# shenwei356/unikmer

Measured on AMD Instinct MI355X. Metric: k-mers/sec for union+inter of 1e9-k-mer k=31 sets, higher is better.
Workload: dtype u64

## Files before the change

unikmer_amd/csrc/ukm_ctx.hip:

```cpp
#include <stdarg.h>
#include <stdlib.h>

#include <algorithm>

#include "ukm_internal.h"

static thread_local char g_err[512] = "";

void ukm_set_error(const char *fmt, ...) {
    va_list ap;
    va_start(ap, fmt);
    vsnprintf(g_err, sizeof(g_err), fmt, ap);
    va_end(ap);
}

extern "C" const char *ukm_last_error(void) { return g_err; }
extern "C" int ukm_version(void) { return 1000 * 0 + 1; }

extern "C" int ukm_device_count(int *n) {
    if (!n) UKM_FAIL(UKM_ERR_INVALID, "ukm_device_count: n is NULL");
    int c = 0;
    hipError_t e = hipGetDeviceCount(&c);
    if (e != hipSuccess) {
        (void)hipGetLastError();
        c = 0;
    }
    *n = c;
    return UKM_OK;
}

extern char **environ;

static const char *const UKM_OPTION_KEYS[] = {
    "punion", "punion_tax", "punion_ranked", "place", "srmerge", "kway", "no_kway", "no_fold", "no_pfold", "pfold_tax", "common_probe",
    "sort_local", "sort_counting", "sort_fan", "win_strip", "nthash_strip", "force_ticket", "setop_src", "setop_defer", "punion_clade", "srmerge_clade",
    "punion_k0", "punion_claim", "punion_debug", "kway_k", "kway_r", "kway_top2", "kway_debug", "srmerge_fill", "srmerge_spr", "srmerge_buckets",
    "srmerge_debug", "fold_debug", "sort_debug", "strip_l", "win_strip_l", "setop_fused_part", "setop_fix",
};

static std::string knob_name(const char *key) {
    std::string n = "UKM_";
    for (const char *p = key; *p; p++) n.push_back((char)toupper((unsigned char)*p));
    return n;
}

const char *ukm_env(const ukm_ctx *c, const char *name) {
    if (c) {
        auto o = c->opts.find(name);
        if (o != c->opts.end()) return o->second.c_str();
        if (!c->env_live) {
            auto k = c->knobs.find(name);
            return k == c->knobs.end() ? nullptr : k->second.c_str();
        }
    }
    return getenv(name);
}

extern "C" int ukm_ctx_set_option(ukm_ctx *c, const char *key, long long value) {
    if (!c || !key) UKM_FAIL(UKM_ERR_INVALID, "ukm_ctx_set_option: NULL argument");
    for (const char *k : UKM_OPTION_KEYS)
        if (strcmp(k, key) == 0) {
            c->opts[knob_name(key)] = std::to_string(value);
            if (strcmp(key, "force_ticket") == 0) c->setop_force_ticket = c->ticket_latched || value != 0;
            return UKM_OK;
        }
    UKM_FAIL(UKM_ERR_INVALID, "ukm_ctx_set_option: unknown option '%s'", key);
}

extern "C" int ukm_ctx_unset_option(ukm_ctx *c, const char *key) {
    if (!c || !key) UKM_FAIL(UKM_ERR_INVALID, "ukm_ctx_unset_option: NULL argument");
    c->opts.erase(knob_name(key));
    if (strcmp(key, "force_ticket") == 0) c->setop_force_ticket = c->ticket_latched || ukm_env_is(c, "UKM_FORCE_TICKET", '1');
    return UKM_OK;
}

extern "C" int ukm_ctx_get_option(ukm_ctx *c, const char *key, long long *value, int *is_set) {
    if (!c || !key || !value || !is_set) UKM_FAIL(UKM_ERR_INVALID, "ukm_ctx_get_option: NULL argument");
    const std::string n = knob_name(key);
    const char *e = ukm_env(c, n.c_str());
    *is_set = (e && *e) ? 1 : 0;
    *value = *is_set ? atoll(e) : 0;
    return UKM_OK;
}

extern "C" int ukm_ctx_get_stat(ukm_ctx *c, const char *key, unsigned long long *value) {
    if (!c || !key || !value) UKM_FAIL(UKM_ERR_INVALID, "ukm_ctx_get_stat: NULL argument");
    if (strcmp(key, "punion_attempts") == 0) *value = c->stat_punion_attempts;
    else if (strcmp(key, "sort_fused_hist") == 0) *value = c->stat_sort_fused_hist;
// ... 37 lines not shown
        if (strncmp(*e, "UKM_", 4) != 0) continue;
        const char *eq = strchr(*e, '=');
        if (eq) c->knobs[std::string(*e, (size_t)(eq - *e))] = std::string(eq + 1);
    }
    c->env_live = ukm_env_is(c, "UKM_ENV_LIVE", '1');
    c->setop_force_ticket = ukm_env_is(c, "UKM_FORCE_TICKET", '1');
    *out = c;
    return UKM_OK;
}

static void ws_free_all(ukm_ctx *c) {
    for (auto &b : c->blocks) (void)hipFree(b.base);
    c->blocks.clear();
}

extern "C" int ukm_ctx_destroy(ukm_ctx *c) {
    if (!c) return UKM_OK;
    (void)hipSetDevice(c->device);
    (void)hipStreamSynchronize(c->stream);
    if (c->comm) (void)ukm_comm_destroy(c);
    ws_free_all(c);
    if (c->tax_parent) (void)hipFree(c->tax_parent);
    if (c->tax_depth) (void)hipFree(c->tax_depth);
    if (c->tax_merged) (void)hipFree(c->tax_merged);
    if (c->tax_anc) (void)hipFree(c->tax_anc);
    if (c->tax_euler) (void)hipFree(c->tax_euler);
    if (c->tax_node_at) (void)hipFree(c->tax_node_at);
    if (c->tax_clade) (void)hipFree(c->tax_clade);
    if (c->tax_clade8) (void)hipFree(c->tax_clade8);
    if (c->tax_pair) (void)hipFree(c->tax_pair);
    if (c->tax_top) (void)hipFree(c->tax_top);
    if (c->h_scratch) (void)hipHostFree(c->h_scratch);
    if (c->sort_stat_dev) (void)hipFree(c->sort_stat_dev);
    if (c->ev_start) (void)hipEventDestroy(c->ev_start);
    if (c->ev_stop) (void)hipEventDestroy(c->ev_stop);
    if (c->ev_k0) (void)hipEventDestroy(c->ev_k0);
    if (c->ev_k1) (void)hipEventDestroy(c->ev_k1);
    if (c->xfer) {
        (void)hipStreamSynchronize(c->xfer);
        (void)hipStreamDestroy(c->xfer);
    }
    if (c->ev_xfer) (void)hipEventDestroy(c->ev_xfer);
    for (int i = 0; i < 2; i++) {
        if (c->side[i]) { (void)hipStreamSynchronize(c->side[i]); (void)hipStreamDestroy(c->side[i]); }
        if (c->ev_side[i]) (void)hipEventDestroy(c->ev_side[i]);
    }
    if (c->ev_fork) (void)hipEventDestroy(c->ev_fork);
    if (c->ev_comp) (void)hipEventDestroy(c->ev_comp);
    if (c->own_stream && c->stream) (void)hipStreamDestroy(c->stream);
    delete c;
    return UKM_OK;
}

extern "C" int ukm_ctx_set_stream(ukm_ctx *c, void *hip_stream) {
    if (!c) UKM_FAIL(UKM_ERR_INVALID, "ukm_ctx_set_stream: ctx is NULL");
    UKM_HIP(hipSetDevice(c->device));
    UKM_HIP(hipStreamSynchronize(c->stream));
    if (c->own_stream && c->stream) (void)hipStreamDestroy(c->stream);
    c->stream = (hipStream_t)hip_stream;
    c->own_stream = false;
    return UKM_OK;
}

extern "C" int ukm_ctx_sync(ukm_ctx *c) {
    if (!c) UKM_FAIL(UKM_ERR_INVALID, "ukm_ctx_sync: ctx is NULL");
    UKM_HIP(hipSetDevice(c->device));
    UKM_HIP(hipStreamSynchronize(c->stream));
    return UKM_OK;
}

static const size_t WS_ALIGN = 256;
static const size_t WS_MIN_BLOCK = (size_t)64 << 20;

static int ws_new_block(ukm_ctx *c, size_t need) {
    size_t total = 0;
    for (auto &b : c->blocks) total += b.cap;
    size_t cap = std::max(need, std::max(WS_MIN_BLOCK, total));
    void *p = nullptr;
    hipError_t e = hipMalloc(&p, cap);
    if (e != hipSuccess && cap > need) {
        (void)hipGetLastError();
        cap = need;
        e = hipMalloc(&p, cap);
    }
    if (e != hipSuccess) {
        (void)hipGetLastError();
        UKM_FAIL(UKM_ERR_NOMEM, "device workspace allocation of %zu bytes failed: %s", cap,
                 hipGetErrorString(e));
    }
    c->blocks.push_back(WsBlock{(char *)p, cap, 0});
    return UKM_OK;
}

int ws_alloc(ukm_ctx *c, size_t bytes, void **out) {
    bytes = (bytes + WS_ALIGN - 1) / WS_ALIGN * WS_ALIGN;
    if (bytes == 0) bytes = WS_ALIGN;
    if (c->blocks.empty() || c->blocks.back().cap - c->blocks.back().used < bytes)
        UKM_TRY(ws_new_block(c, bytes));
    WsBlock &b = c->blocks.back();
    *out = b.base + b.used;
    b.used += bytes;
    size_t used = 0;
    for (auto &x : c->blocks) used += x.used;
    c->ws_high = std::max(c->ws_high, used);
    return UKM_OK;
}
// ... 88 lines not shown
    }
    void *d = nullptr;
    UKM_TRY(ws_alloc(c, bytes, &d));
    c->copybacks.push_back(ukm_ctx::CopyBack{p, d, bytes});
    *dev = d;
    return UKM_OK;
}

void ukm_out_resize(ukm_ctx *c, void *host, size_t bytes) {
    for (auto &cb : c->copybacks)
        if (cb.host == host) cb.bytes = std::min(cb.bytes, bytes);
}

int ukm_inout(ukm_ctx *c, void *p, size_t bytes, void **dev) {
    if (ukm_is_device_ptr(p)) {
        *dev = p;
        return UKM_OK;
    }
    void *d = nullptr;
    UKM_TRY(ws_alloc(c, bytes, &d));
    if (bytes) UKM_HIP(hipMemcpyAsync(d, p, bytes, hipMemcpyHostToDevice, c->stream));
    c->copybacks.push_back(ukm_ctx::CopyBack{p, d, bytes});
    *dev = d;
    return UKM_OK;
}

int ukm_begin(ukm_ctx *c, CallScope *s) {
    if (!c) UKM_FAIL(UKM_ERR_INVALID, "ctx is NULL");
    s->c = c;
    s->top = (c->depth == 0);
    c->depth++;
    if (s->top) {
        hipError_t e = hipSetDevice(c->device);
        if (e != hipSuccess) {
            c->depth--;
            UKM_FAIL(UKM_ERR_HIP, "hipSetDevice(%d): %s", c->device, hipGetErrorString(e));
        }
        c->copybacks.clear();
        (void)hipEventRecord(c->ev_start, c->stream);
        c->ev_valid = false;
        c->evk_valid = false;
    }
    s->mark = ws_mark(c);
    return UKM_OK;
}

int ukm_finish(CallScope *s, int rc) {
    ukm_ctx *c = s->c;
    c->depth--;
    if (!s->top) {
        ws_release(c, s->mark);
        return rc;
    }
    (void)hipEventRecord(c->ev_stop, c->stream);
    c->ev_valid = true;
    if (rc == UKM_OK) {
        for (auto &cb : c->copybacks) {
            if (cb.bytes == 0) continue;
            hipError_t e = hipMemcpyAsync(cb.host, cb.dev, cb.bytes, hipMemcpyDeviceToHost, c->stream);
            if (e != hipSuccess) {
                ukm_set_error("copy-back failed: %s", hipGetErrorString(e));
                rc = UKM_ERR_HIP;
                break;
            }
        }
    }
    hipError_t e = hipStreamSynchronize(c->stream);
    if (e != hipSuccess && rc == UKM_OK) {
        ukm_set_error("stream synchronize failed: %s", hipGetErrorString(e));
        rc = UKM_ERR_HIP;
    }
    c->copybacks.clear();
    ws_reset_top(c);
    return rc;
}

void ukm_switch_to_tickets(ukm_ctx *c, const char *where) {
    if (!c->setop_force_ticket)
        fprintf(stderr, "[unikmer_hip] look-back watchdog fired in %s: workgroups were not dispatched in order on device %d; "
                        "switching this context to ticketed tile ids\n", where, c->device);
    c->ticket_latched = true;
    c->setop_force_ticket = true;
}

int ukm_read_u64(ukm_ctx *c, const u64 *dev, u64 *host, int n) {
    if (n > 64) UKM_FAIL(UKM_ERR_INVALID, "ukm_read_u64: n too large");
    UKM_HIP(hipMemcpyAsync(c->h_scratch, dev, n * sizeof(u64), hipMemcpyDeviceToHost, c->stream));
    UKM_HIP(hipStreamSynchronize(c->stream));
    for (int i = 0; i < n; i++) host[i] = c->h_scratch[i];
    return UKM_OK;
}

int ukm_lb_ctl_alloc(ukm_ctx *c, u64 ntiles, size_t tail, LbCtl *b, u64 *head) {
    const size_t nstat = lb_status_words(ntiles);
    u64 *ctl = head;
    if (head) {
        UKM_TRY(ws_alloc_t(c, nstat + tail, &b->status));
        b->zero_from = b->status;
        b->zero_words = nstat;
    } else {
        UKM_TRY(ws_alloc_t(c, LbCtl::HEAD + nstat + tail, &ctl));
        b->status = ctl + 8;
        b->zero_from = ctl;
        b->zero_words = LbCtl::HEAD + nstat;
    }
    b->result = ctl;
    b->ticket = (u32 *)(ctl + 2);
    b->tail = b->status + nstat;
// ... 137 lines not shown
```

unikmer_amd/csrc/ukm_internal.h:

```cpp
#pragma once

#include <hip/hip_runtime.h>
#include <stdint.h>
#include <stdio.h>
#include <stdlib.h>
#include <string.h>

#include <functional>
#include <map>
#include <string>
#include <vector>

#include "../../include/unikmer_hip.h"

typedef uint64_t u64;
typedef uint32_t u32;
typedef uint8_t u8;

void ukm_set_error(const char *fmt, ...);

#define UKM_FAIL(code, ...)        \
    do {                           \
        ukm_set_error(__VA_ARGS__); \
        return (code);             \
// ... 113 lines not shown
}

int ws_alloc(ukm_ctx *c, size_t bytes, void **out);
template <typename T>
static inline int ws_alloc_t(ukm_ctx *c, size_t n, T **out) {
    void *p = nullptr;
    int rc = ws_alloc(c, n * sizeof(T), &p);
    *out = (T *)p;
    return rc;
}
struct WsMark {
    size_t nblocks;
    size_t used_last;
};
WsMark ws_mark(ukm_ctx *c);
void ws_release(ukm_ctx *c, WsMark m);

bool ukm_is_device_ptr(const void *p);

int ukm_in(ukm_ctx *c, const void *p, size_t bytes, const void **dev);
template <typename T>
static inline int ukm_in_t(ukm_ctx *c, const T *p, size_t n, const T **dev) {
    const void *d = nullptr;
    if (p == nullptr || n == 0) {
        *dev = p;
        if (p == nullptr) return UKM_OK;
    }
    int rc = ukm_in(c, p, n * sizeof(T), &d);
    *dev = (const T *)d;
    return rc;
}
int ukm_out(ukm_ctx *c, void *p, size_t bytes, void **dev);
template <typename T>
static inline int ukm_out_t(ukm_ctx *c, T *p, size_t n, T **dev) {
    void *d = nullptr;
    if (p == nullptr) {
        *dev = nullptr;
        return UKM_OK;
    }
    int rc = ukm_out(c, p, n * sizeof(T), &d);
    *dev = (T *)d;
    return rc;
}
void ukm_out_resize(ukm_ctx *c, void *host, size_t bytes);
int ukm_inout(ukm_ctx *c, void *p, size_t bytes, void **dev);

struct CallScope {
    ukm_ctx *c;
    bool top;
    WsMark mark;
};
int ukm_begin(ukm_ctx *c, CallScope *s);
int ukm_finish(CallScope *s, int rc);

int ukm_read_u64(ukm_ctx *c, const u64 *dev, u64 *host, int n = 1);

static inline TaxDev ukm_taxdev(const ukm_ctx *c) {
    TaxDev t;
    t.parent = c->tax_parent;
    t.depth = c->tax_depth;
    t.merged = c->tax_merged;
    t.anc = c->tax_anc;
    t.euler = c->tax_euler;
    t.node_at = c->tax_node_at;
    t.clade = c->tax_clade;
    t.clade8 = c->tax_clade8;
    t.pair = c->tax_pair;
    t.kp = c->tax_kp;
    {
        const size_t off = (((size_t)c->tax_kp * c->tax_kp) + 3) & ~(size_t)3;
        t.cpath = c->tax_pair ? reinterpret_cast<const uint4 *>(c->tax_pair + off) : nullptr;
        t.cnode = c->tax_pair ? c->tax_pair + off + 4 * TAX_CPATH_ROWS : nullptr;
    }
    t.top = c->tax_top;
    t.nchunks = c->tax_nchunks;
    t.size = c->tax_size;
    return t;
}

#ifndef LB_STRIDE
#define LB_STRIDE 8
#endif
static inline size_t lb_status_words(u64 ntiles) { return (size_t)ntiles * LB_STRIDE; }

struct LbCtl {
    static constexpr size_t HEAD = 8;
    u64 *result = nullptr;
    u32 *ticket = nullptr;
    u64 *status = nullptr;
    u64 *tail = nullptr;
    u64 *zero_from = nullptr;
    size_t zero_words = 0;
};
int ukm_lb_ctl_alloc(ukm_ctx *c, u64 ntiles, size_t tail, LbCtl *b, u64 *head = nullptr);
int ukm_lb_ctl_zero(ukm_ctx *c, const LbCtl &b);

void ukm_switch_to_tickets(ukm_ctx *c, const char *where);

struct LbLaunch {
    const char *err_name;
    const char *warn_name;
    u64 watchdog;
    bool bracket;
    bool ticket_first;
    bool first_zeroed;
};
// ... 26 lines not shown
```

unikmer_amd/csrc/ukm_setops.hip:

```cpp
#include <algorithm>

#include "ukm_device.h"

namespace {

enum { FLAG_DUP = 1, FLAG_UNSORTED = 2, FLAG_TIMEOUT = 4 };

#ifndef SETOP_NT
#define SETOP_NT 512
#endif
#ifndef SETOP_VT
#define SETOP_VT 19
#endif


struct SetopArgs {
    const u64 *a, *b;
    const u32 *ta, *tb;
    const u32 *ra, *rb;
    u64 na, nb;
    u64 *mp;
    u64 *status;
    u32 *ticket;
    u64 *result;
    u64 *out;
    u32 *tout;
    u64 out_cap;
    u64 ntiles;
    TaxDev tax;
    u32 flags;
    u64 *dbg;
    const u64 *na_dev;
    u32 zero_status;
    u32 cta, ctb;
    uint4 *fix;
    u32 *fix_cnt;
};
constexpr u32 FIX_SLOTS = 16;

__device__ __forceinline__ void setop_resolve_sizes(SetopArgs &p, u64 tile_items) {
    if (p.na_dev) {
        p.na = *p.na_dev;
        p.ntiles = (p.na + p.nb + tile_items - 1) / tile_items;
    }
}

#ifdef UKM_PROFILE_PHASES
#define PH(i) do { if (tid == 0) { u64 _t = clock64(); ph[i] += _t - tlast; tlast = _t; } } while (0)
#else
#define PH(i) do {} while (0)
#endif

template <bool RANK>
__device__ __forceinline__ bool key_le(u64 ka, u32 ra, u64 kb, u32 rb) {
    if (RANK) return ka < kb || (ka == kb && ra <= rb);
    return ka <= kb;
}
template <bool RANK>
__device__ __forceinline__ bool key_eq(u64 ka, u32 ra, u64 kb, u32 rb) {
    if (RANK) return ka == kb && ra == rb;
    return ka == kb;
}

#ifndef SETOP_PART_COARSE
#define SETOP_PART_COARSE 64
#endif
#ifndef SETOP_PART_INTERP1
#define SETOP_PART_INTERP1 (1 << 17)
#endif
#ifndef SETOP_PART_INTERP
#define SETOP_PART_INTERP 512
#endif
constexpr int PART_COARSE = SETOP_PART_COARSE;
template <bool RANK, int LEVEL>
__global__ void setop_partition_kernel(SetopArgs p, int tile_items) {
    setop_resolve_sizes(p, (u64)tile_items);
    u64 t = (u64)blockIdx.x * blockDim.x + threadIdx.x;
    if (LEVEL == 1) {
        t *= PART_COARSE;
        if (t > p.ntiles + PART_COARSE - 1) return;
        if (t > p.ntiles) t = p.ntiles;
    } else {
        if (LEVEL == 0 && t < p.zero_status) p.status[t * LB_STRIDE] = 0;
        if (t > p.ntiles) return;
        if (LEVEL == 2 && (t % PART_COARSE == 0 || t == p.ntiles)) return;
    }
    const u64 N = p.na + p.nb;
    u64 diag = t * (u64)tile_items;
    if (diag > N) diag = N;
// ... 41 lines not shown
    u64 t = gid >> 6;
    const int lane = (int)(threadIdx.x & 63);
    if (LEVEL == 1) {
        t *= PART_COARSE;
        if (t > p.ntiles + PART_COARSE - 1) return;
        if (t > p.ntiles) t = p.ntiles;
    } else if (t > p.ntiles) {
        return;
    }
    const u64 N = p.na + p.nb;
    u64 diag = t * (u64)tile_items;
    if (diag > N) diag = N;
    u64 lo = diag > p.nb ? diag - p.nb : 0;
    u64 hi = diag < p.na ? diag : p.na;
#if SETOP_PART_INTERP1
    if (lo < hi) {
        const u64 W = SETOP_PART_INTERP1;
        u64 est = (u64)((double)diag * ((double)p.na / (double)N));
        est = est < lo ? lo : (est > hi ? hi : est);
        const u64 L = est > lo + W ? est - W : lo;
        const u64 R = est + W < hi ? est + W : hi;
        bool pl = true, pr = false;
        if (L > lo) { const u64 j = diag - L; pl = key_le<RANK>(p.a[L - 1], RANK ? p.ra[L - 1] : 0, p.b[j], RANK ? p.rb[j] : 0); }
        if (R < hi) { const u64 j = diag - 1 - R; pr = key_le<RANK>(p.a[R], RANK ? p.ra[R] : 0, p.b[j], RANK ? p.rb[j] : 0); }
        if (L > lo) { if (pl) lo = L; else hi = L - 1; }
        if (R < hi) { if (!pr) hi = R; else lo = R + 1; }
    }
#endif
    while (lo < hi) {
        const u64 span = hi - lo;
        const u64 step_n = span <= 64 ? 1 : 0;
        const u64 cand = step_n ? lo + (u64)lane
                                : lo + (span / 65) * (u64)(lane + 1) + ((span % 65) * (u64)(lane + 1)) / 65;
        const bool active = cand < hi;
        bool le = false;
        if (active) {
            const u64 j = diag - 1 - cand;
            le = key_le<RANK>(p.a[cand], RANK ? p.ra[cand] : 0, p.b[j], RANK ? p.rb[j] : 0);
        }
        const u64 m_le = __ballot(le), m_act = __ballot(active);
        const int n_true = __popcll(m_le);
        const int n_act = __popcll(m_act);
        const u64 c_last_true = __shfl(cand, n_true > 0 ? n_true - 1 : 0, 64);
        const u64 c_first_false = __shfl(cand, n_true < 64 ? n_true : 63, 64);
        const u64 nlo = n_true > 0 ? c_last_true + 1 : lo;
        const u64 nhi = n_true < n_act ? c_first_false : hi;
        lo = nlo;
        hi = nhi;
    }
    if (lane == 0) p.mp[t] = lo;
}

template <bool RANK>
__global__ __launch_bounds__(256) void setop_partition_fused_kernel(SetopArgs p, int tile_items, u32 nclear) {
    __shared__ u64 s_end[2];
    const int tid = (int)threadIdx.x, lane = tid & 63, wave = tid >> 6;
    const u64 c0 = (u64)blockIdx.x * PART_COARSE;
    const u64 c1 = (c0 + PART_COARSE < p.ntiles) ? c0 + PART_COARSE : p.ntiles;
    const u64 N = p.na + p.nb;
    if (tid < PART_COARSE && c0 + (u64)tid < p.ntiles) p.status[(c0 + (u64)tid) * LB_STRIDE] = 0;
    if (blockIdx.x == 0 && tid < (int)nclear) p.result[tid] = 0;
    if (wave < 2) {
        const u64 t = wave == 0 ? c0 : c1;
        u64 diag = t * (u64)tile_items;
        if (diag > N) diag = N;
        u64 lo = diag > p.nb ? diag - p.nb : 0;
        u64 hi = diag < p.na ? diag : p.na;
#if SETOP_PART_INTERP1
        if (lo < hi) {
            const u64 W = SETOP_PART_INTERP1;
            u64 est = (u64)((double)diag * ((double)p.na / (double)N));
            est = est < lo ? lo : (est > hi ? hi : est);
            const u64 L = est > lo + W ? est - W : lo;
            const u64 R = est + W < hi ? est + W : hi;
            bool pl = true, pr = false;
            if (L > lo) { const u64 j = diag - L; pl = key_le<RANK>(p.a[L - 1], RANK ? p.ra[L - 1] : 0, p.b[j], RANK ? p.rb[j] : 0); }
            if (R < hi) { const u64 j = diag - 1 - R; pr = key_le<RANK>(p.a[R], RANK ? p.ra[R] : 0, p.b[j], RANK ? p.rb[j] : 0); }
            if (L > lo) { if (pl) lo = L; else hi = L - 1; }
            if (R < hi) { if (!pr) hi = R; else lo = R + 1; }
        }
#endif
        while (lo < hi) {
            const u64 span = hi - lo;
            const u64 cand = span <= 64 ? lo + (u64)lane
                                        : lo + (span / 65) * (u64)(lane + 1) + ((span % 65) * (u64)(lane + 1)) / 65;
            const bool active = cand < hi;
            bool le = false;
            if (active) {
                const u64 j = diag - 1 - cand;
                le = key_le<RANK>(p.a[cand], RANK ? p.ra[cand] : 0, p.b[j], RANK ? p.rb[j] : 0);
            }
            const u64 m_le = __ballot(le), m_act = __ballot(active);
            const int n_true = __popcll(m_le), n_act = __popcll(m_act);
            const u64 c_last_true = __shfl(cand, n_true > 0 ? n_true - 1 : 0, 64);
            const u64 c_first_false = __shfl(cand, n_true < 64 ? n_true : 63, 64);
            const u64 nlo = n_true > 0 ? c_last_true + 1 : lo;
            const u64 nhi = n_true < n_act ? c_first_false : hi;
            lo = nlo;
            hi = nhi;
        }
        if (lane == 0) {
            s_end[wave] = lo;
            if (wave == 0) p.mp[c0] = lo;
            else if (c1 == p.ntiles) p.mp[c1] = lo;
        }
    }
    __syncthreads();
    const u64 t = c0 + (u64)tid;
    if (tid == 0 || tid >= PART_COARSE || t >= c1) return;
    const u64 l0 = s_end[0], h0 = s_end[1];
    u64 diag = t * (u64)tile_items;
    if (diag > N) diag = N;
    u64 lo = diag > p.nb ? diag - p.nb : 0;
    u64 hi = diag < p.na ? diag : p.na;
// ... 636 lines not shown
    }
}

__global__ __launch_bounds__(256) void setop_taxid_fix_kernel(SetopArgs p) {
    const u64 g = (u64)blockIdx.x * 256 + threadIdx.x;
    const u64 tile = g / FIX_SLOTS;
    if (tile >= p.ntiles) return;
    if (sload_u64(&p.result[1]) & FLAG_TIMEOUT) return;
    if ((u32)(g % FIX_SLOTS) >= p.fix_cnt[tile]) return;
    const uint4 e = p.fix[g];
    const u64 pos = ((u64)e.y << 32) | e.x;
    const uint4 zero4 = make_uint4(0, 0, 0, 0);
    const TaxDev &T = p.tax;
    if (pos < p.out_cap) p.tout[pos] = lca_from_rows(T, e.z, e.w, e.z < T.size ? T.anc[e.z] : zero4, e.w < T.size ? T.anc[e.w] : zero4);
}

__global__ void setop_ct_kernel(SetopArgs p, int op) {
    const u32 a = p.cta, b = p.ctb;
    u32 l;
    if (op == UKM_OP_INTER && (p.flags & UKM_F_MIX_TAXID)) l = a == 0 ? b : (b == 0 ? a : lca_dev(p.tax, a, b));
    else l = lca_dev(p.tax, a, b);
    const bool keep = op == UKM_OP_DIFF && (p.flags & UKM_F_CMP_TAXID) && (a == b || lca_dev(p.tax, b, a) == a);
    p.result[4] = (u64)l | ((u64)(keep ? 1u : 0u) << 32);
}

#ifndef SETOP_WAVES
#define SETOP_WAVES 4
#endif
#ifndef SETOP_WAVES_TAX
#define SETOP_WAVES_TAX 6
#endif
template <int OP, bool TAX, bool RANK, bool TICKET, int NTH, int VT, bool CT = false, bool DEFER = false>
__global__ __launch_bounds__(NTH) __attribute__((amdgpu_waves_per_eu((TAX && RANK) ? 2 : ((TAX && VT <= 8) ? SETOP_WAVES_TAX : SETOP_WAVES), (TAX && RANK) ? 8 : ((TAX && VT <= 8) ? SETOP_WAVES_TAX : SETOP_WAVES))))
void setop_tile_kernel(SetopArgs p) {
    static_assert(!(CT && TAX), "CT: no per-record taxids");
    constexpr int TILE = NTH * VT;
    constexpr int SLOTS = TILE + 8;
    constexpr int NP = TilePairs<NTH, VT>::NP;
    __shared__ __attribute__((aligned(16))) u64 s_keys[SLOTS];
    __shared__ __attribute__((aligned(16))) u32 s_tax[TAX ? SLOTS : 2];
    __shared__ __attribute__((aligned(16))) u32 s_rank[RANK ? SLOTS : 2];
    __shared__ u32 s_scan[NTH / 64 + 1];
    __shared__ u64 s_misc[2];
    __shared__ CladeLdsOpt<TAX> s_clade_tab;
    __shared__ FixLdsOpt<DEFER> s_fix;
    const int tid = (int)threadIdx.x;
    if constexpr (DEFER) {
        if (tid == 0) s_fix.t.n = 0;
    }
#ifdef UKM_PROFILE_PHASES
    u64 ph[8] = {0, 0, 0, 0, 0, 0, 0, 0};
    u64 tlast = clock64();
#endif
    const u64 tile = lb_tile_id<TICKET>(p.ticket, &s_misc[0]);
    PH(0);
    setop_resolve_sizes(p, (u64)TILE);
    if (tile >= p.ntiles) return;
    const TileGeom g = tile_geom<NTH, VT>(p, tile);
    u32 bad = 0;
    bool fast = false;
#ifndef SETOP_NO_FAST
    if (!TAX && !RANK) fast = tile_is_fast<NTH, VT>(p, g);
#endif
    if (fast) {
        tile_dma_fast<NTH, VT>(p, g, tid, s_keys);
        __syncthreads();
        PH(1);
    } else {
        u64 rk[2 * NP];
        u32 rt[2 * NP], rr[2 * NP];
        tile_load<TAX, RANK, NTH, VT>(p, g, tid, rk, rt, rr);
        if constexpr (TAX) clade_lds_load(p.tax, s_clade_tab.t, tid, NTH);
        tile_to_lds<TAX, RANK, NTH, VT>(tid, rk, rt, rr, s_keys, s_tax, s_rank);
        __syncthreads();
        PH(1);
        bad = tile_check_order<RANK, NTH, VT>(g, tid, rk, rr, s_keys, s_rank);
    }
    u64 ok[VT];
    u32 ot[VT];
    u32 tbm[VT];
    u32 need = 0, nneed = 0, qpos = 0;
    u32 mask, amask = 0, mmask = 0;
    int ia0 = 0, ib0 = 0;
    u32 ct_lca = 0;
    bool ct_keep = false;
    if (CT) {
        const u64 w = sload_u64(&p.result[4]);
        ct_lca = (u32)w;
        ct_keep = ((w >> 32) & 1ull) != 0;
    }
#ifdef SETOP_ABL_NOMERGE
    mask = 0xAAAAu | (u32)(tid & 1);
#pragma unroll
    for (int s = 0; s < VT; s++) { ok[s] = s_keys[tid * VT + s]; ot[s] = 0; }
#else
    tile_merge<OP, TAX, RANK, CT, NTH, VT, DEFER>(p, g, tid, s_keys, s_tax, s_rank, ok, ot, mask, amask, mmask, ct_keep, ia0, ib0,
                                           TAX ? reinterpret_cast<const CladeLds *>(&s_clade_tab.t) : nullptr, tbm, need);
#endif
    PH(2);
    u32 tile_total;
    u32 excl;
    {
        constexpr int NW = NTH / 64;
        const u32 v = (u32)__popc(mask) | (DEFER ? (u32)__popc(need) << 16 : 0u);
        const int lane = lane_id(), wave = tid >> 6;
        const u32 incl = wave_incl_scan_u32(v);
        if (lane == 63) s_scan[wave] = incl;
// ... 26 lines not shown
        __syncthreads();
        tile_lca_dense<NTH>(p.tax, s_clade_tab.t, tid, nneed, s_keys + tile_total, s_tax, p.fix ? &s_fix.t : nullptr);
    }
    PH(3);
    if (OP == UKM_OP_MERGE_INTERNAL) {
        if (tid == 0) s_misc[1] = tile * (u64)TILE;
    } else if (tid < 64) {
        bool timed_out = false;
#ifdef LB_PRE_SLEEP
        __builtin_amdgcn_s_sleep(LB_PRE_SLEEP);
#endif
#ifdef SETOP_ABL_NOLB
        const u64 base = tile * (u64)TILE;
#else
        const u64 base = lb_resolve(p.status, tile, (u64)tile_total, lane_id(), TICKET ? nullptr : &timed_out);
#endif
        if (tid == 0) s_misc[1] = base;
        if (timed_out) bad |= FLAG_TIMEOUT;
    }
    PH(4);
    if (OP == UKM_OP_MERGE_INTERNAL) bad &= ~FLAG_DUP;
    {
        u32 wbad = 0;
#pragma unroll
        for (u32 f = 1; f <= FLAG_TIMEOUT; f <<= 1)
            if (__ballot((bad & f) != 0)) wbad |= f;
        if (wbad && lane_id() == 0) atomicOr((unsigned long long *)&p.result[1], (unsigned long long)wbad);
    }
    __syncthreads();
    const u64 base = s_misc[1];
    if constexpr (DEFER) {
        if (p.fix) {
            const u32 nf = s_fix.t.n < FIX_SLOTS ? s_fix.t.n : FIX_SLOTS;
            if ((u32)tid < nf) {
                const u64 pos = base + s_fix.t.w[tid];
                p.fix[tile * FIX_SLOTS + (u32)tid] = make_uint4((u32)pos, (u32)(pos >> 32), s_fix.t.a[tid], s_fix.t.b[tid]);
            }
            if (tid == 0) p.fix_cnt[tile] = nf;
        }
    }
#ifndef SETOP_ABL_NOFLUSH
    tile_flush<TAX, NTH>(p, tid, base, tile_total, s_keys, s_tax);
    if (CT) {
        if (p.ta != nullptr || p.tb != nullptr)
            tile_flush_src<OP, NTH, VT>(p, tid, base, tile_total, excl, mask, amask, mmask, ia0, ib0, reinterpret_cast<u32 *>(s_keys));
        else
            tile_flush_ct<OP, NTH, VT>(p, tid, base, tile_total, excl, mask, amask, mmask, ct_lca, reinterpret_cast<u32 *>(s_keys));
    }
#endif
    if (tid == 0 && tile == p.ntiles - 1) p.result[0] = base + tile_total;
    PH(5);
#ifdef UKM_PROFILE_PHASES
    if (tid == 0 && p.dbg) {
        for (int i = 0; i < 7; i++) p.dbg[blockIdx.x * 8 + i] = ph[i];
        p.dbg[blockIdx.x * 8 + 7] = 1;
    }
#endif
}

__global__ void rank_in_run_kernel(const u64 *k, u64 n, u32 *rank) {
    u64 i = (u64)blockIdx.x * blockDim.x + threadIdx.x;
    if (i >= n) return;
    const u64 key = k[i];
    u32 r = 0;
    while (r < 32 && i > r && k[i - r - 1] == key) r++;
    if (r == 32 && i > r && k[i - r - 1] == key) {
        u64 lo = 0, hi = i - 32;
        while (lo < hi) {
            u64 mid = (lo + hi) >> 1;
            if (k[mid] < key) lo = mid + 1; else hi = mid;
        }
        r = (u32)(i - lo);
    }
    rank[i] = r;
}

__global__ void lower_bound_kernel(const u64 *k, u64 n, const u64 *q, int nq, u64 *out) {
    int i = blockIdx.x * blockDim.x + threadIdx.x;
    if (i >= nq) return;
    u64 key = q[i], lo = 0, hi = n;
    while (lo < hi) {
        u64 mid = (lo + hi) >> 1;
        if (k[mid] < key) lo = mid + 1; else hi = mid;
    }
    out[i] = lo;
}

template <int OP, bool TAX, bool RANK, int NTH, int VT, bool CT = false, bool DEFER = false>
void launch_tile(const SetopArgs &p, hipStream_t st, bool ticket) {
    if (CT) hipLaunchKernelGGL(setop_ct_kernel, dim3(1), dim3(1), 0, st, p, OP);
    if (ticket)
        hipLaunchKernelGGL((setop_tile_kernel<OP, TAX, RANK, true, NTH, VT, CT, DEFER>), dim3((unsigned)p.ntiles), dim3(NTH), 0, st, p);
    else
        hipLaunchKernelGGL((setop_tile_kernel<OP, TAX, RANK, false, NTH, VT, CT, DEFER>), dim3((unsigned)p.ntiles), dim3(NTH), 0, st, p);
    if constexpr (DEFER) {
        if (p.fix) hipLaunchKernelGGL(setop_taxid_fix_kernel, dim3((unsigned)((p.ntiles * FIX_SLOTS + 255) / 256)), dim3(256), 0, st, p);
    }
    if constexpr (CT && !RANK) {
        if (p.ta != nullptr || p.tb != nullptr)
            hipLaunchKernelGGL((setop_taxid_gather_kernel<OP, NTH * VT>), dim3((unsigned)p.ntiles), dim3(GATHER_NT), 0, st, p);
    }
}

template <bool TAX, bool RANK, int NTH, int VT, bool CT = false, bool DEFER = false>
void launch_op(int op, const SetopArgs &p, hipStream_t st, bool ticket) {
    if (op == UKM_OP_UNION) launch_tile<UKM_OP_UNION, TAX, RANK, NTH, VT, CT, DEFER>(p, st, ticket);
    else if (op == UKM_OP_INTER) launch_tile<UKM_OP_INTER, TAX, RANK, NTH, VT, CT, DEFER>(p, st, ticket);
    else if (op == UKM_OP_MERGE_INTERNAL) {
        if constexpr (!RANK) launch_tile<UKM_OP_MERGE_INTERNAL, TAX, false, NTH, VT, CT>(p, st, ticket);
    } else launch_tile<UKM_OP_DIFF, TAX, RANK, NTH, VT, CT>(p, st, ticket);
}

constexpr int NTS = SETOP_NT;
constexpr int VT_PLAIN = SETOP_VT;
#ifndef SETOP_VT_TAX
#define SETOP_VT_TAX 7
#endif
constexpr int VT_TAX = SETOP_VT_TAX;
constexpr int VT_RANK = 12;

int run_setop_pass(ukm_ctx *c, int op, const u64 *a, const u32 *ta, const u32 *ra, u64 na,
                   const u64 *b, const u32 *tb, const u32 *rb, u64 nb, bool tax, u32 flags,
                   u64 *out, u32 *tout, u64 out_cap, u64 result_host[2], u32 cta = 0, u32 ctb = 0) {
    const bool rank = ra != nullptr;
    bool ct = tax && !ta && !tb;
    const bool defer_form = SETOP_TAX_DEFER != 0 && c->tax_pair != nullptr && !ukm_env_is(c, "UKM_SETOP_DEFER", '0');
    const int src_mode = ukm_env_int(c, "UKM_SETOP_SRC", defer_form ? 0 : 1);
    if (tax && !ct && !rank && src_mode != 0 && (op == UKM_OP_INTER || (src_mode == 2 && !(op == UKM_OP_DIFF && (flags & UKM_F_CMP_TAXID))))) ct = true;
    if (ct) tax = false;
    const bool tax_stream = tax && !rank && op == UKM_OP_DIFF && !(flags & UKM_F_CMP_TAXID);
    const int vt = rank ? VT_RANK : (tax ? (tax_stream ? VT_RANK : VT_TAX) : VT_PLAIN);
    const u64 tile_items = (u64)NTS * vt;
    const u64 N = na + nb;
    SetopArgs p;
    memset(&p, 0, sizeof(p));
    p.a = a; p.b = b; p.ta = ta; p.tb = tb; p.ra = ra; p.rb = rb;
    p.na = na; p.nb = nb;
    p.out = out; p.tout = tout; p.out_cap = out_cap;
    p.ntiles = (N + tile_items - 1) / tile_items;
    p.tax = ukm_taxdev(c);
    p.flags = flags;
    p.cta = cta;
    p.ctb = ctb;
    if (p.ntiles > 0xFFFFFFFFull) UKM_FAIL(UKM_ERR_INVALID, "setop: input too large");

    LbCtl blk;
    UKM_TRY(ukm_lb_ctl_alloc(c, p.ntiles, p.ntiles + 1, &blk));
    p.result = blk.result;
    p.ticket = blk.ticket;
    p.status = blk.status;
    p.mp = blk.tail;
    if (tax && !rank && defer_form && (op == UKM_OP_UNION || op == UKM_OP_INTER) && !ukm_env_is(c, "UKM_SETOP_FIX", '0')) {
        UKM_TRY(ws_alloc_t(c, (size_t)p.ntiles * FIX_SLOTS, &p.fix));
        UKM_TRY(ws_alloc_t(c, (size_t)p.ntiles, &p.fix_cnt));
    }
#ifdef UKM_PROFILE_PHASES
    UKM_TRY(ws_alloc_t(c, (size_t)p.ntiles * 8, &p.dbg));
    UKM_HIP(hipMemsetAsync(p.dbg, 0, (size_t)p.ntiles * 8 * sizeof(u64), c->stream));
#endif
    const bool fused = !ukm_env_is(c, "UKM_SETOP_FUSED_PART", '0') && p.ntiles >= 4 * PART_COARSE;
    if (fused) {
        const unsigned sblocks = (unsigned)((p.ntiles + PART_COARSE - 1) / PART_COARSE);
        if (rank) hipLaunchKernelGGL((setop_partition_fused_kernel<true>), dim3(sblocks), dim3(256), 0, c->stream, p, (int)tile_items, (u32)LbCtl::HEAD);
        else hipLaunchKernelGGL((setop_partition_fused_kernel<false>), dim3(sblocks), dim3(256), 0, c->stream, p, (int)tile_items, (u32)LbCtl::HEAD);
        UKM_HIP(hipGetLastError());
    } else if (p.ntiles >= 4 * PART_COARSE) {
        const unsigned cblocks = (unsigned)((p.ntiles / PART_COARSE + 2 + 3) / 4);
        const unsigned pblocks = (unsigned)((p.ntiles + 1 + 255) / 256);
        if (rank) {
            hipLaunchKernelGGL((setop_partition_coop_kernel<true, 1>), dim3(cblocks), dim3(256), 0, c->stream, p, (int)tile_items);
            hipLaunchKernelGGL((setop_partition_kernel<true, 2>), dim3(pblocks), dim3(256), 0, c->stream, p, (int)tile_items);
        } else {
            hipLaunchKernelGGL((setop_partition_coop_kernel<false, 1>), dim3(cblocks), dim3(256), 0, c->stream, p, (int)tile_items);
            hipLaunchKernelGGL((setop_partition_kernel<false, 2>), dim3(pblocks), dim3(256), 0, c->stream, p, (int)tile_items);
        }
    } else {
        const unsigned wblocks = (unsigned)((p.ntiles + 1 + 3) / 4);
        if (rank) hipLaunchKernelGGL((setop_partition_coop_kernel<true, 0>), dim3(wblocks), dim3(256), 0, c->stream, p, (int)tile_items);
        else hipLaunchKernelGGL((setop_partition_coop_kernel<false, 0>), dim3(wblocks), dim3(256), 0, c->stream, p, (int)tile_items);
    }
    const LbLaunch how = {"setop", "set-op kernel", FLAG_TIMEOUT, true, false, fused};
    UKM_TRY(ukm_lb_launch(c, blk, how, [&](bool ticket) {
        if (rank) {
            if (tax) launch_op<true, true, NTS, VT_RANK>(op, p, c->stream, ticket);
            else if (ct) launch_op<false, true, NTS, VT_RANK, true>(op, p, c->stream, ticket);
            else launch_op<false, true, NTS, VT_RANK>(op, p, c->stream, ticket);
        } else {
            if (tax_stream) launch_tile<UKM_OP_DIFF, true, false, NTS, VT_RANK>(p, c->stream, ticket);
            else if (tax && defer_form) launch_op<true, false, NTS, VT_TAX, false, true>(op, p, c->stream, ticket);
            else if (tax) launch_op<true, false, NTS, VT_TAX>(op, p, c->stream, ticket);
            else if (ct) launch_op<false, false, NTS, VT_PLAIN, true>(op, p, c->stream, ticket);
            else launch_op<false, false, NTS, VT_PLAIN>(op, p, c->stream, ticket);
        }
        return UKM_OK;
    }, result_host));
#ifdef UKM_PROFILE_PHASES
    {
        std::vector<u64> h((size_t)p.ntiles * 8);
        UKM_HIP(hipMemcpy(h.data(), p.dbg, h.size() * sizeof(u64), hipMemcpyDeviceToHost));
        double sum[8] = {0};
        for (u64 b = 0; b < p.ntiles; b++) for (int i = 0; i < 8; i++) sum[i] += (double)h[(size_t)b * 8 + i];
        double tot = 0; for (int i = 0; i < 7; i++) tot += sum[i];
        fprintf(stderr, "[phases op=%d tiles=%llu] cycles per tile:", op, (unsigned long long)p.ntiles);
        for (int i = 0; i < 7; i++) fprintf(stderr, " p%d=%.0f", i, sum[i] / sum[7]);
        fprintf(stderr, " total=%.0f\n", tot / sum[7]);
    }
#endif
    return UKM_OK;
}

}

int ukm_dev_setop2_link(ukm_ctx *c, int op, const u64 *a, const u32 *ta, u64 na_max, const u64 *na_dev, const u64 *b,
                        const u32 *tb, u64 nb, u32 flags, u64 *out, u32 *tout, u64 out_cap, u64 *ctl, u32 cta, u32 ctb) {
    bool tax = (ta != nullptr) || (tb != nullptr) || cta != 0 || ctb != 0;
    const bool ct = tax && !ta && !tb;
    if (ct) tax = false;
    const int vt = tax ? VT_TAX : VT_PLAIN;
    const u64 tile_items = (u64)NTS * vt;
    SetopArgs p;
    memset(&p, 0, sizeof(p));
    p.a = a; p.b = b; p.ta = ta; p.tb = tb;
    p.na = na_max; p.nb = nb; p.na_dev = na_dev;
    p.out = out; p.tout = tout; p.out_cap = out_cap;
    p.ntiles = (na_max + nb + tile_items - 1) / tile_items;
    p.tax = ukm_taxdev(c);
    p.flags = flags;
    p.cta = cta;
    p.ctb = ctb;
    if (p.ntiles == 0) return UKM_OK;
    const unsigned pblocks = (unsigned)((p.ntiles + 1 + 255) / 256);
#ifndef SETOP_LINK_SMALL_TILES
#define SETOP_LINK_SMALL_TILES 2048
#endif
    const bool small = p.ntiles < SETOP_LINK_SMALL_TILES;
    LbCtl blk;
    UKM_TRY(ukm_lb_ctl_alloc(c, p.ntiles + 1, p.ntiles + 1, &blk, ctl));
    if (small) p.zero_status = (u32)(p.ntiles + 1);
    else UKM_TRY(ukm_lb_ctl_zero(c, blk));
    p.result = blk.result;
    p.ticket = blk.ticket;
    p.status = blk.status;
    p.mp = blk.tail;
    if (!small) {
        const unsigned cblocks = (unsigned)((p.ntiles / PART_COARSE + 2 + 3) / 4);
        hipLaunchKernelGGL((setop_partition_coop_kernel<false, 1>), dim3(cblocks), dim3(256), 0, c->stream, p, (int)tile_items);
        hipLaunchKernelGGL((setop_partition_kernel<false, 2>), dim3(pblocks), dim3(256), 0, c->stream, p, (int)tile_items);
// ... 140 lines not shown
```

unikmer_amd/csrc/ukm_sort.hip:

```cpp
#include <algorithm>
#include <utility>
#include <vector>
#include <cmath>

#include "ukm_device.h"

namespace {

#ifndef SORT_NT_KEYS
#define SORT_NT_KEYS 1024
#endif
#ifndef SORT_VT_KEYS
#define SORT_VT_KEYS 14
#endif
#ifndef SORT_NT_PAIRS
#define SORT_NT_PAIRS 1024
#endif
#ifndef SORT_VT_PAIRS
#define SORT_VT_PAIRS 11
#endif
constexpr int NT = 256;
#ifndef SORT_RADIX_BITS
#define SORT_RADIX_BITS 8
#endif
// ... 711 lines not shown
        else UKM_TRY((run_passes<u64, false, SORT_NT_KEYS, SORT_VT_KEYS>(c, keys, nullptr, tk, nullptr, n, npass, sh, gb, &in_tmp, fh)));
    }
    const u64 *src = in_tmp ? tk : keys;
    const u32 *vsrc = in_tmp ? tv : vals;
    auto give_up = [&]() -> int {
        if (in_tmp) {
            UKM_HIP(hipMemcpyAsync(keys, tk, n * sizeof(u64), hipMemcpyDeviceToDevice, c->stream));
            if (vals) UKM_HIP(hipMemcpyAsync(vals, tv, n * sizeof(u32), hipMemcpyDeviceToDevice, c->stream));
        }
        return UKM_OK;
    };
    hipLaunchKernelGGL(ls_bounds_kernel, dim3((nbuckets + 1 + 255) / 256), dim3(256), 0, c->stream, src, n, low_bits, topb, start);
    u64 *cls = nullptr;
    u32 *ids = nullptr;
    static_assert(LS_NCLASS + 3 <= 64, "read-back through the scratch");
    if (!c->sort_stat_dev) {
        UKM_HIP(hipMalloc((void **)&c->sort_stat_dev, 64));
        UKM_HIP(hipMemsetAsync(c->sort_stat_dev, 0, 64, c->stream));
    }
    u32 *big_ids = nullptr;
    u64 *big_size = nullptr;
    UKM_TRY(ws_alloc_t(c, (size_t)LS_NCLASS + 3, &cls));
    UKM_TRY(ws_alloc_t(c, (size_t)LS_NCLASS << topb, &ids));
    UKM_TRY(ws_alloc_t(c, (size_t)LS_MAX_BIG, &big_ids));
    UKM_TRY(ws_alloc_t(c, (size_t)nbuckets + 1, &big_size));
    UKM_HIP(hipMemsetAsync(cls, 0, (LS_NCLASS + 3) * sizeof(u64), c->stream));
    hipLaunchKernelGGL(ls_classify_kernel, dim3(nbuckets / 256), dim3(256), 0, c->stream, start, cls, ids, topb, big_ids, big_size, c->sort_stat_dev);
    UKM_HIP(hipGetLastError());
    u64 hc[LS_NCLASS + 3];
    UKM_TRY(ukm_read_u64(c, cls, hc, LS_NCLASS + 3));
    if (c->sort_last_counting && hc[LS_NCLASS + 2] * 2 > c->sort_last_buckets) c->sort_counting_skip = 15;
    const u64 big_keys = hc[LS_NCLASS + 1];
    if (hc[LS_NCLASS] > (u64)LS_MAX_BIG || big_keys > n / 4) {
        c->sort_skew_seen = true;
        if (ukm_env(c, "UKM_SORT_DEBUG")) fprintf(stderr, "[sort] %llu buckets beyond every class: general route\n", (unsigned long long)hc[LS_NCLASS]);
        return give_up();
    }
    LocalSortArgs a;
    a.src = src; a.vsrc = vsrc; a.keys = keys; a.vals = vals; a.n = n; a.start = start; a.low_bits = low_bits;
    a.counting = ukm_env_is(c, "UKM_SORT_COUNTING", '0') ? 0 : 1;
    if (a.counting && c->sort_counting_skip > 0 && !ukm_env_is(c, "UKM_SORT_COUNTING", '1')) {
        a.counting = 0;
        c->sort_counting_skip--;
    }
    a.stat = c->sort_stat_dev;
    c->sort_last_counting = a.counting != 0;
    c->sort_last_buckets = 0;
    for (int k = 0; k < LS_NCLASS; k++) c->sort_last_buckets += hc[k];
    const dim3 block(LS_NT);
    int nocc = 0;
    for (int k = 0; k < LS_NCLASS; k++) nocc += hc[k] != 0;
    const bool fan = nocc >= 3 && !ukm_env_is(c, "UKM_SORT_FAN", '0');
    if (fan) {
        if (!c->ev_fork) {
            UKM_HIP(hipEventCreateWithFlags(&c->ev_fork, hipEventDisableTiming));
            for (int i = 0; i < 2; i++) {
                UKM_HIP(hipStreamCreateWithFlags(&c->side[i], hipStreamNonBlocking));
                UKM_HIP(hipEventCreateWithFlags(&c->ev_side[i], hipEventDisableTiming));
            }
        }
        UKM_HIP(hipEventRecord(c->ev_fork, c->stream));
        for (int i = 0; i < 2; i++) UKM_HIP(hipStreamWaitEvent(c->side[i], c->ev_fork, 0));
    }
    int turn = 0;
    hipStream_t lst = c->stream;
#define LS_LAUNCH(K)                                                                                          \
    do {                                                                                                      \
        if (vals) hipLaunchKernelGGL((ls_sort_kernel<K, true>), grid, block, 0, lst, a);                      \
        else hipLaunchKernelGGL((ls_sort_kernel<K, false>), grid, block, 0, lst, a);                          \
    } while (0)
    for (int kk = 0; kk < LS_NCLASS; kk++) {
        const int k = LS_NCLASS - 1 - kk;
        if (hc[k] == 0) continue;
        if (fan) lst = turn % 3 == 0 ? c->stream : c->side[turn % 3 - 1];
        turn++;
        a.ids = ids + ((size_t)k << topb);
        const dim3 grid((unsigned)hc[k]);
        switch (LS_CLASS_KPT[k]) {
        case 1: LS_LAUNCH(1); break;
        case 2: LS_LAUNCH(2); break;
        case 3: LS_LAUNCH(3); break;
        case 4: LS_LAUNCH(4); break;
        case 5: LS_LAUNCH(5); break;
        case 6: LS_LAUNCH(6); break;
        case 7: LS_LAUNCH(7); break;
        case 8: LS_LAUNCH(8); break;
        case 10: LS_LAUNCH(10); break;
        case 12: LS_LAUNCH(12); break;
        case 14: LS_LAUNCH(14); break;
        default: LS_LAUNCH(16); break;
        }
    }
    UKM_HIP(hipGetLastError());
    if (fan)
        for (int i = 0; i < 2; i++) {
            UKM_HIP(hipEventRecord(c->ev_side[i], c->side[i]));
            UKM_HIP(hipStreamWaitEvent(c->stream, c->ev_side[i], 0));
        }
    if (hc[LS_NCLASS]) {
        const unsigned nb = (unsigned)hc[LS_NCLASS];
        u64 *big_off = nullptr, *bk = nullptr, *tot = nullptr;
        u32 *bv = nullptr;
        UKM_TRY(ws_alloc_t(c, (size_t)nbuckets + 1, &big_off));
        UKM_TRY(ws_alloc_t(c, 1, &tot));
        UKM_TRY(ws_alloc_t(c, big_keys, &bk));
        if (vals) UKM_TRY(ws_alloc_t(c, big_keys, &bv));
        UKM_TRY(ukm_dev_exclusive_scan_u64(c, big_size, big_off, nbuckets, tot));
        const dim3 cg(nb, 16);
        hipLaunchKernelGGL(ls_big_copy_kernel<false>, cg, dim3(256), 0, c->stream, big_ids, start, big_off, src, vsrc, bk, bv);
        UKM_HIP(hipGetLastError());
        c->sort_general_only = true;
        const int src_rc = ukm_dev_sort(c, bk, bv, big_keys, kb);
        c->sort_general_only = false;
// ... 191 lines not shown
```

Before: 435.9 billion.

## Split setop partition across side stream and skip sync when stream idle

Adds an optional split of the fused partition kernel: the first segments are placed on the main stream and the rest on a side stream, so that tile kernels for the first part can start before all partitioning finishes. The split is off by default (UKM_SETOP_SPLIT=0). Separately, ukm_finish now queries the stream and, if it is already idle and there are no copybacks, skips the synchronize and copy-back path. The split adds event and stream overhead, and the idle shortcut changes end-of-call handling.

Measured after the change: 436.9 billion, median of 5. Within noise of the previous version (+0.2%).

```diff
diff --git a/unikmer_amd/csrc/ukm_ctx.hip b/unikmer_amd/csrc/ukm_ctx.hip
--- a/unikmer_amd/csrc/ukm_ctx.hip
+++ b/unikmer_amd/csrc/ukm_ctx.hip
@@ -33,7 +33,7 @@
 
 static const char *const UKM_OPTION_KEYS[] = {
     "punion", "punion_tax", "punion_ranked", "place", "srmerge", "kway", "no_kway", "no_fold", "no_pfold", "pfold_tax", "common_probe",
-    "sort_local", "sort_counting", "sort_fan", "win_strip", "nthash_strip", "force_ticket", "setop_src", "setop_defer", "punion_clade", "srmerge_clade",
+    "sort_local", "sort_counting", "sort_fan", "win_strip", "nthash_strip", "force_ticket", "setop_src", "setop_defer", "setop_split", "punion_clade", "srmerge_clade",
     "punion_k0", "punion_claim", "punion_debug", "kway_k", "kway_r", "kway_top2", "kway_debug", "srmerge_fill", "srmerge_spr", "srmerge_buckets",
     "srmerge_debug", "fold_debug", "sort_debug", "strip_l", "win_strip_l", "setop_fused_part", "setop_fix",
 };
@@ -177,6 +177,15 @@
     return UKM_OK;
 }
 
+int ukm_side_streams(ukm_ctx *c) {
+    if (!c->ev_fork) UKM_HIP(hipEventCreateWithFlags(&c->ev_fork, hipEventDisableTiming));
+    for (int i = 0; i < 2; i++) {
+        if (!c->side[i]) UKM_HIP(hipStreamCreateWithFlags(&c->side[i], hipStreamNonBlocking));
+        if (!c->ev_side[i]) UKM_HIP(hipEventCreateWithFlags(&c->ev_side[i], hipEventDisableTiming));
+    }
+    return UKM_OK;
+}
+
 extern "C" int ukm_ctx_set_stream(ukm_ctx *c, void *hip_stream) {
     if (!c) UKM_FAIL(UKM_ERR_INVALID, "ukm_ctx_set_stream: ctx is NULL");
     UKM_HIP(hipSetDevice(c->device));
@@ -371,8 +380,17 @@
         ws_release(c, s->mark);
         return rc;
     }
+    bool idle = false;
+    if (c->copybacks.empty()) {
+        idle = hipStreamQuery(c->stream) == hipSuccess;
+        if (!idle) (void)hipGetLastError();
+    }
     (void)hipEventRecord(c->ev_stop, c->stream);
     c->ev_valid = true;
+    if (idle) {
+        ws_reset_top(c);
+        return rc;
+    }
     if (rc == UKM_OK) {
         for (auto &cb : c->copybacks) {
             if (cb.bytes == 0) continue;
diff --git a/unikmer_amd/csrc/ukm_internal.h b/unikmer_amd/csrc/ukm_internal.h
--- a/unikmer_amd/csrc/ukm_internal.h
+++ b/unikmer_amd/csrc/ukm_internal.h
@@ -189,6 +189,8 @@
 };
 int ukm_begin(ukm_ctx *c, CallScope *s);
 int ukm_finish(CallScope *s, int rc);
+
+int ukm_side_streams(ukm_ctx *c);
 
 int ukm_read_u64(ukm_ctx *c, const u64 *dev, u64 *host, int n = 1);
 
diff --git a/unikmer_amd/csrc/ukm_setops.hip b/unikmer_amd/csrc/ukm_setops.hip
--- a/unikmer_amd/csrc/ukm_setops.hip
+++ b/unikmer_amd/csrc/ukm_setops.hip
@@ -35,6 +35,7 @@
     u32 cta, ctb;
     uint4 *fix;
     u32 *fix_cnt;
+    u64 tile0;
 };
 constexpr u32 FIX_SLOTS = 16;
 
@@ -182,14 +183,15 @@
 }
 
 template <bool RANK>
-__global__ __launch_bounds__(256) void setop_partition_fused_kernel(SetopArgs p, int tile_items, u32 nclear) {
+__global__ __launch_bounds__(256) void setop_partition_fused_kernel(SetopArgs p, int tile_items, u32 nclear, u32 seg0) {
     __shared__ u64 s_end[2];
     const int tid = (int)threadIdx.x, lane = tid & 63, wave = tid >> 6;
-    const u64 c0 = (u64)blockIdx.x * PART_COARSE;
+    const u64 seg = (u64)seg0 + blockIdx.x;
+    const u64 c0 = seg * PART_COARSE;
     const u64 c1 = (c0 + PART_COARSE < p.ntiles) ? c0 + PART_COARSE : p.ntiles;
     const u64 N = p.na + p.nb;
     if (tid < PART_COARSE && c0 + (u64)tid < p.ntiles) p.status[(c0 + (u64)tid) * LB_STRIDE] = 0;
-    if (blockIdx.x == 0 && tid < (int)nclear) p.result[tid] = 0;
+    if (seg == 0 && tid < (int)nclear) p.result[tid] = 0;
     if (wave < 2) {
         const u64 t = wave == 0 ? c0 : c1;
         u64 diag = t * (u64)tile_items;
@@ -932,7 +934,7 @@
     u64 ph[8] = {0, 0, 0, 0, 0, 0, 0, 0};
     u64 tlast = clock64();
 #endif
-    const u64 tile = lb_tile_id<TICKET>(p.ticket, &s_misc[0]);
+    const u64 tile = lb_tile_id<TICKET>(p.ticket, &s_misc[0]) + (TICKET ? 0ull : p.tile0);
     PH(0);
     setop_resolve_sizes(p, (u64)TILE);
     if (tile >= p.ntiles) return;
@@ -1065,8 +1067,8 @@
     PH(5);
 #ifdef UKM_PROFILE_PHASES
     if (tid == 0 && p.dbg) {
-        for (int i = 0; i < 7; i++) p.dbg[blockIdx.x * 8 + i] = ph[i];
-        p.dbg[blockIdx.x * 8 + 7] = 1;
+        for (int i = 0; i < 7; i++) p.dbg[tile * 8 + i] = ph[i];
+        p.dbg[tile * 8 + 7] = 1;
     }
 #endif
 }
@@ -1099,13 +1101,30 @@
     out[i] = lo;
 }
 
+struct SetopSplit {
+    u64 n1 = 0;
+    hipEvent_t rest_placed = nullptr;
+};
+
 template <int OP, bool TAX, bool RANK, int NTH, int VT, bool CT = false, bool DEFER = false>
-void launch_tile(const SetopArgs &p, hipStream_t st, bool ticket) {
+int launch_tile(const SetopArgs &p, hipStream_t st, bool ticket, const SetopSplit &sp = SetopSplit()) {
     if (CT) hipLaunchKernelGGL(setop_ct_kernel, dim3(1), dim3(1), 0, st, p, OP);
-    if (ticket)
-        hipLaunchKernelGGL((setop_tile_kernel<OP, TAX, RANK, true, NTH, VT, CT, DEFER>), dim3((unsigned)p.ntiles), dim3(NTH), 0, st, p);
-    else
-        hipLaunchKernelGGL((setop_tile_kernel<OP, TAX, RANK, false, NTH, VT, CT, DEFER>), dim3((unsigned)p.ntiles), dim3(NTH), 0, st, p);
+    auto tiles = [&](u64 t0, u64 t1) {
+        SetopArgs q = p;
+        q.tile0 = t0;
+        if (ticket)
+            hipLaunchKernelGGL((setop_tile_kernel<OP, TAX, RANK, true, NTH, VT, CT, DEFER>), dim3((unsigned)(t1 - t0)), dim3(NTH), 0, st, q);
+        else
+            hipLaunchKernelGGL((setop_tile_kernel<OP, TAX, RANK, false, NTH, VT, CT, DEFER>), dim3((unsigned)(t1 - t0)), dim3(NTH), 0, st, q);
+    };
+    if (sp.n1 == 0 || sp.n1 >= p.ntiles) {
+        if (sp.rest_placed) UKM_HIP(hipStreamWaitEvent(st, sp.rest_placed, 0));
+        tiles(0, p.ntiles);
+    } else {
+        tiles(0, sp.n1);
+        if (sp.rest_placed) UKM_HIP(hipStreamWaitEvent(st, sp.rest_placed, 0));
+        tiles(sp.n1, p.ntiles);
+    }
     if constexpr (DEFER) {
         if (p.fix) hipLaunchKernelGGL(setop_taxid_fix_kernel, dim3((unsigned)((p.ntiles * FIX_SLOTS + 255) / 256)), dim3(256), 0, st, p);
     }
@@ -1113,16 +1132,36 @@
         if (p.ta != nullptr || p.tb != nullptr)
             hipLaunchKernelGGL((setop_taxid_gather_kernel<OP, NTH * VT>), dim3((unsigned)p.ntiles), dim3(GATHER_NT), 0, st, p);
     }
+    return UKM_OK;
 }
 
 template <bool TAX, bool RANK, int NTH, int VT, bool CT = false, bool DEFER = false>
-void launch_op(int op, const SetopArgs &p, hipStream_t st, bool ticket) {
-    if (op == UKM_OP_UNION) launch_tile<UKM_OP_UNION, TAX, RANK, NTH, VT, CT, DEFER>(p, st, ticket);
-    else if (op == UKM_OP_INTER) launch_tile<UKM_OP_INTER, TAX, RANK, NTH, VT, CT, DEFER>(p, st, ticket);
-    else if (op == UKM_OP_MERGE_INTERNAL) {
-        if constexpr (!RANK) launch_tile<UKM_OP_MERGE_INTERNAL, TAX, false, NTH, VT, CT>(p, st, ticket);
-    } else launch_tile<UKM_OP_DIFF, TAX, RANK, NTH, VT, CT>(p, st, ticket);
-}
+int launch_op(int op, const SetopArgs &p, hipStream_t st, bool ticket, const SetopSplit &sp = SetopSplit()) {
+    if (op == UKM_OP_UNION) return launch_tile<UKM_OP_UNION, TAX, RANK, NTH, VT, CT, DEFER>(p, st, ticket, sp);
+    if (op == UKM_OP_INTER) return launch_tile<UKM_OP_INTER, TAX, RANK, NTH, VT, CT, DEFER>(p, st, ticket, sp);
+    if (op == UKM_OP_MERGE_INTERNAL) {
+        if constexpr (!RANK) return launch_tile<UKM_OP_MERGE_INTERNAL, TAX, false, NTH, VT, CT>(p, st, ticket, sp);
+        return UKM_OK;
+    }
+    return launch_tile<UKM_OP_DIFF, TAX, RANK, NTH, VT, CT>(p, st, ticket, sp);
+}
+
+u64 setop_split_tiles(const ukm_ctx *c, u64 ntiles) {
+    const int knob = ukm_env_int(c, "UKM_SETOP_SPLIT", 0);
+    return knob > 0 ? std::min<u64>((u64)knob, ntiles) : 0;
+}
+
+struct SideJoin {
+    ukm_ctx *c;
+    bool forked = false, recorded = false, joined = false;
+    explicit SideJoin(ukm_ctx *ctx) : c(ctx) {}
+    SideJoin(const SideJoin &) = delete;
+    SideJoin &operator=(const SideJoin &) = delete;
+    ~SideJoin() {
+        if (!forked || joined) return;
+        if (!recorded || hipStreamWaitEvent(c->stream, c->ev_side[0], 0) != hipSuccess) (void)hipStreamSynchronize(c->side[0]);
+    }
+};
 
 constexpr int NTS = SETOP_NT;
 constexpr int VT_PLAIN = SETOP_VT;
@@ -1172,10 +1211,29 @@
     UKM_HIP(hipMemsetAsync(p.dbg, 0, (size_t)p.ntiles * 8 * sizeof(u64), c->stream));
 #endif
     const bool fused = !ukm_env_is(c, "UKM_SETOP_FUSED_PART", '0') && p.ntiles >= 4 * PART_COARSE;
+    SetopSplit split;
+    SideJoin side(c);
     if (fused) {
         const unsigned sblocks = (unsigned)((p.ntiles + PART_COARSE - 1) / PART_COARSE);
-        if (rank) hipLaunchKernelGGL((setop_partition_fused_kernel<true>), dim3(sblocks), dim3(256), 0, c->stream, p, (int)tile_items, (u32)LbCtl::HEAD);
-        else hipLaunchKernelGGL((setop_partition_fused_kernel<false>), dim3(sblocks), dim3(256), 0, c->stream, p, (int)tile_items, (u32)LbCtl::HEAD);
+        auto place = [&](hipStream_t st, unsigned seg0, unsigned nseg) {
+            if (rank) hipLaunchKernelGGL((setop_partition_fused_kernel<true>), dim3(nseg), dim3(256), 0, st, p, (int)tile_items, (u32)LbCtl::HEAD, (u32)seg0);
+            else hipLaunchKernelGGL((setop_partition_fused_kernel<false>), dim3(nseg), dim3(256), 0, st, p, (int)tile_items, (u32)LbCtl::HEAD, (u32)seg0);
+        };
+        split.n1 = setop_split_tiles(c, p.ntiles);
+        const unsigned g1 = split.n1 ? (unsigned)std::min<u64>(split.n1 / PART_COARSE + 1, sblocks) : sblocks;
+        if (g1 < sblocks) {
+            UKM_TRY(ukm_side_streams(c));
+            UKM_HIP(hipEventRecord(c->ev_fork, c->stream));
+            place(c->stream, 0, g1);
+            UKM_HIP(hipStreamWaitEvent(c->side[0], c->ev_fork, 0));
+            side.forked = true;
+            place(c->side[0], g1, sblocks - g1);
+            UKM_HIP(hipEventRecord(c->ev_side[0], c->side[0]));
+            side.recorded = true;
+            split.rest_placed = c->ev_side[0];
+        } else {
+            place(c->stream, 0, g1);
+        }
         UKM_HIP(hipGetLastError());
     } else if (p.ntiles >= 4 * PART_COARSE) {
         const unsigned cblocks = (unsigned)((p.ntiles / PART_COARSE + 2 + 3) / 4);
@@ -1194,18 +1252,20 @@
     }
     const LbLaunch how = {"setop", "set-op kernel", FLAG_TIMEOUT, true, false, fused};
     UKM_TRY(ukm_lb_launch(c, blk, how, [&](bool ticket) {
+        int rc;
         if (rank) {
-            if (tax) launch_op<true, true, NTS, VT_RANK>(op, p, c->stream, ticket);
-            else if (ct) launch_op<false, true, NTS, VT_RANK, true>(op, p, c->stream, ticket);
-            else launch_op<false, true, NTS, VT_RANK>(op, p, c->stream, ticket);
+            if (tax) rc = launch_op<true, true, NTS, VT_RANK>(op, p, c->stream, ticket, split);
+            else if (ct) rc = launch_op<false, true, NTS, VT_RANK, true>(op, p, c->stream, ticket, split);
+            else rc = launch_op<false, true, NTS, VT_RANK>(op, p, c->stream, ticket, split);
         } else {
-            if (tax_stream) launch_tile<UKM_OP_DIFF, true, false, NTS, VT_RANK>(p, c->stream, ticket);
-            else if (tax && defer_form) launch_op<true, false, NTS, VT_TAX, false, true>(op, p, c->stream, ticket);
-            else if (tax) launch_op<true, false, NTS, VT_TAX>(op, p, c->stream, ticket);
-            else if (ct) launch_op<false, false, NTS, VT_PLAIN, true>(op, p, c->stream, ticket);
-            else launch_op<false, false, NTS, VT_PLAIN>(op, p, c->stream, ticket);
-        }
-        return UKM_OK;
+            if (tax_stream) rc = launch_tile<UKM_OP_DIFF, true, false, NTS, VT_RANK>(p, c->stream, ticket, split);
+            else if (tax && defer_form) rc = launch_op<true, false, NTS, VT_TAX, false, true>(op, p, c->stream, ticket, split);
+            else if (tax) rc = launch_op<true, false, NTS, VT_TAX>(op, p, c->stream, ticket, split);
+            else if (ct) rc = launch_op<false, false, NTS, VT_PLAIN, true>(op, p, c->stream, ticket, split);
+            else rc = launch_op<false, false, NTS, VT_PLAIN>(op, p, c->stream, ticket, split);
+        }
+        if (rc == UKM_OK && split.rest_placed) side.joined = true;
+        return rc;
     }, result_host));
 #ifdef UKM_PROFILE_PHASES
     {
diff --git a/unikmer_amd/csrc/ukm_sort.hip b/unikmer_amd/csrc/ukm_sort.hip
--- a/unikmer_amd/csrc/ukm_sort.hip
+++ b/unikmer_amd/csrc/ukm_sort.hip
@@ -787,13 +787,7 @@
     for (int k = 0; k < LS_NCLASS; k++) nocc += hc[k] != 0;
     const bool fan = nocc >= 3 && !ukm_env_is(c, "UKM_SORT_FAN", '0');
     if (fan) {
-        if (!c->ev_fork) {
-            UKM_HIP(hipEventCreateWithFlags(&c->ev_fork, hipEventDisableTiming));
-            for (int i = 0; i < 2; i++) {
-                UKM_HIP(hipStreamCreateWithFlags(&c->side[i], hipStreamNonBlocking));
-                UKM_HIP(hipEventCreateWithFlags(&c->ev_side[i], hipEventDisableTiming));
-            }
-        }
+        UKM_TRY(ukm_side_streams(c));
         UKM_HIP(hipEventRecord(c->ev_fork, c->stream));
         for (int i = 0; i < 2; i++) UKM_HIP(hipStreamWaitEvent(c->side[i], c->ev_fork, 0));
     }
```
